# lalitkrajendran/photon

Hardware: AMD Instinct MI355X
Metric: Mrays/sec, 1e7-ray 256^3 BOS render (higher is better)
Workload: dtype f32

## Files before the change

photon_amd/csrc/device_volume_coop.hpp:

```cpp
#pragma once
#include "../../include/photon_philox.h"
#include "device_volume.hpp"

namespace photon {

enum PathSlot : int {
    PS_C_COHERENT,
    PS_C_HIT_CELL,
    PS_C_CELL_IN_TILE,
    PS_C_FETCH_UP,
    PS_C_FETCH_DOWN,
    PS_C_TILE_CLAMPED,
    PS_C_INCOHERENT,
    PS_C_INCOHERENT_LANES,
    PS_C_BRICK_PASS,
    PS_C_BRICK_FETCH,
    PS_C_BRICK_REUSED,
    PS_C_BRICK_CLAMPED,
    PS_C_BRICK_LANES,
    PS_C_GATHER_LANES,
    PS_C_SPIN_OUTSIDE,
    PS_C_SPIN_LOW,
    PS_C_SPIN_CAP,
    PS_L_COHERENT,
    PS_L_HIT_A,
    PS_L_HIT_B,
    PS_L_TILE_B_LANES,
    PS_L_FETCH,
    PS_L_FETCH_TWO,
    PS_L_FETCH_TO_B,
    PS_L_FETCH_DOWN,
    PS_L_BASE_AHEAD,
    PS_L_BASE_BEHIND,
    PS_L_TILE_CLAMPED,
    PS_L_NO_FREE_TILE,
    PS_L_OUT_OF_REACH,
    PS_L_MARK_INCOHERENT,
    PS_L_TILES_SKIPPED,
    PS_L_RETRY,
    PS_L_COHERENT_AGAIN,
    PS_L_INCOHERENT,
    PS_L_INCOHERENT_LANES,
    PS_L_BRICK_PASS,
    PS_L_BRICK_FETCH,
    PS_L_BRICK_REUSED,
    PS_L_BRICK_CLAMPED,
    PS_L_BRICK_LANES,
    PS_L_GATHER_LANES,
    PS_L_SPIN_OUTSIDE,
    PS_L_SPIN_CAP,
    PS_L_LOW,
    PS_L_REPAIR_LANES,
    PS_L_KEEP_PREV_LANES,
    PS_COUNT
};
constexpr int kPathSlots = PS_COUNT;
#ifndef PHOTON_PATH_STATS
#define PHOTON_PATH_STATS 0
#endif
#if PHOTON_PATH_STATS
__device__ unsigned long long g_path_stats[kPathSlots];
__device__ __forceinline__ void path_stat(PathSlot k, unsigned long long n = 1) {
    if ((int)(threadIdx.x & 63) == __ffsll((long long)ballot(true)) - 1) atomicAdd(&g_path_stats[k], n);
}
__device__ __forceinline__ void path_stat_if(PathSlot k, bool c) { if (c) path_stat(k); }
__device__ __forceinline__ void path_lanes(PathSlot k, unsigned long long mask) { if (mask != 0) path_stat(k, (unsigned long long)__popcll(mask)); }
#else
#define path_stat(...) ((void)0)
#define path_stat_if(...) ((void)0)
#define path_lanes(...) ((void)0)
#endif

#ifndef PHOTON_BRICK_PASSES
#define PHOTON_BRICK_PASSES 6
#endif
#ifndef PHOTON_LINEAR_TILE_LAYERS
#define PHOTON_LINEAR_TILE_LAYERS 16
#endif
#ifndef PHOTON_LINEAR_TILES
#define PHOTON_LINEAR_TILES 2
#endif
#ifndef PHOTON_TILE_RETRY_MASK
#define PHOTON_TILE_RETRY_MASK 15
#endif
#ifndef PHOTON_BRICK_PITCH
#define PHOTON_BRICK_PITCH 12
#endif
constexpr int kBrickPitch = PHOTON_BRICK_PITCH;
constexpr int kBrickSlab = 8 * kBrickPitch;
#ifndef PHOTON_CUBIC_TILE_LAYERS
#define PHOTON_CUBIC_TILE_LAYERS 7
#endif
constexpr int kCubicTileLayers = PHOTON_CUBIC_TILE_LAYERS;
static_assert(kCubicTileLayers >= 4 && kCubicTileLayers <= 8, "PHOTON_CUBIC_TILE_LAYERS");
template <int INTERP> constexpr int tile_texels() { return INTERP == 2 ? 16 * kCubicTileLayers : PHOTON_LINEAR_TILES * PHOTON_LINEAR_TILE_LAYERS * 4; }
#ifndef PHOTON_SPINS_IN_LDS
#define PHOTON_SPINS_IN_LDS 1
#endif
constexpr int kSpinSlotTexels = PHOTON_SPINS_IN_LDS ? 32 : 0;
template <int INTERP> constexpr int wave_lds_texels() { return tile_texels<INTERP>() + (INTERP == 2 ? 4 : 2) * kBrickSlab + (INTERP == 1 ? kSpinSlotTexels : 0); }
constexpr int kWaveLdsTexels = wave_lds_texels<2>();

template <int RS, int SS>
__device__ __forceinline__ f4 cubic_taps_lds(const f4 *blk, const float (&wx)[4], const float (&wy)[4],
                                             const float (&wz)[4]) {
    float wxy[4][4];
#pragma unroll
    for (int b = 0; b < 4; b++)
#pragma unroll
        for (int a = 0; a < 4; a++) wxy[b][a] = wx[a] * wy[b];
    f4 acc = f4{0, 0, 0, 0}, s = f4{0, 0, 0, 0};
    float w0 = wxy[0][0];
    f4 t[4];
#pragma unroll
    for (int a = 0; a < 4; a++) t[a] = ldtexel(blk + a);
#pragma unroll
    for (int r = 0; r < 16; r++) {
        const int b = r & 3, c = r >> 2;
#pragma unroll
        for (int a = 0; a < 4; a++) {
            const f4 ta = t[a];
            const float w = (a == 0 && b == 0) ? w0 : wxy[b][a];
            if (a == 0 && b == 0) s = f4{w * ta.x, w * ta.y, w * ta.z, w * ta.w};
            else s = f4{fmaf(w, ta.x, s.x), fmaf(w, ta.y, s.y), fmaf(w, ta.z, s.z), fmaf(w, ta.w, s.w)};
            asm volatile("" : "+v"(s.x), "+v"(s.y), "+v"(s.z), "+v"(s.w) : : "memory");
            if (r < 15) t[a] = ldtexel(blk + ((r + 1) >> 2) * SS + ((r + 1) & 3) * RS + a);
            asm volatile("" : "+v"(w0) : : "memory");
        }
        if (b == 3) {
            if (c == 0) acc = f4{wz[0] * s.x, wz[0] * s.y, wz[0] * s.z, wz[0] * s.w};
            else acc = f4{fmaf(wz[c], s.x, acc.x), fmaf(wz[c], s.y, acc.y), fmaf(wz[c], s.z, acc.z), fmaf(wz[c], s.w, acc.w)};
            asm volatile("" : "+v"(acc.x), "+v"(acc.y), "+v"(acc.z), "+v"(acc.w) : : "memory");
        }
    }
    return acc;
}

#define PH_DPP_ROW0 \
    "v_mul_f32_dpp %0, %8, %12 row_newbcast:0 row_mask:0xf bank_mask:0xf\n\t" \
    "v_mul_f32_dpp %1, %9, %12 row_newbcast:0 row_mask:0xf bank_mask:0xf\n\t" \
    "v_mul_f32_dpp %2, %10, %12 row_newbcast:0 row_mask:0xf bank_mask:0xf\n\t" \
    "v_mul_f32_dpp %3, %11, %12 row_newbcast:0 row_mask:0xf bank_mask:0xf\n\t" \
    "v_fmac_f32_dpp %0, %8, %13 row_newbcast:1 row_mask:0xf bank_mask:0xf\n\t" \
    "v_fmac_f32_dpp %1, %9, %13 row_newbcast:1 row_mask:0xf bank_mask:0xf\n\t" \
    "v_fmac_f32_dpp %2, %10, %13 row_newbcast:1 row_mask:0xf bank_mask:0xf\n\t" \
    "v_fmac_f32_dpp %3, %11, %13 row_newbcast:1 row_mask:0xf bank_mask:0xf\n\t" \
    "v_fmac_f32_dpp %0, %8, %14 row_newbcast:2 row_mask:0xf bank_mask:0xf\n\t" \
    "v_fmac_f32_dpp %1, %9, %14 row_newbcast:2 row_mask:0xf bank_mask:0xf\n\t" \
    "v_fmac_f32_dpp %2, %10, %14 row_newbcast:2 row_mask:0xf bank_mask:0xf\n\t" \
    "v_fmac_f32_dpp %3, %11, %14 row_newbcast:2 row_mask:0xf bank_mask:0xf\n\t" \
    "v_fmac_f32_dpp %0, %8, %15 row_newbcast:3 row_mask:0xf bank_mask:0xf\n\t" \
    "v_fmac_f32_dpp %1, %9, %15 row_newbcast:3 row_mask:0xf bank_mask:0xf\n\t" \
    "v_fmac_f32_dpp %2, %10, %15 row_newbcast:3 row_mask:0xf bank_mask:0xf\n\t" \
    "v_fmac_f32_dpp %3, %11, %15 row_newbcast:3 row_mask:0xf bank_mask:0xf\n\t"
#define PH_DPP_ROW1 \
    "v_fmac_f32_dpp %0, %8, %16 row_newbcast:4 row_mask:0xf bank_mask:0xf\n\t" \
    "v_fmac_f32_dpp %1, %9, %16 row_newbcast:4 row_mask:0xf bank_mask:0xf\n\t" \
    "v_fmac_f32_dpp %2, %10, %16 row_newbcast:4 row_mask:0xf bank_mask:0xf\n\t" \
    "v_fmac_f32_dpp %3, %11, %16 row_newbcast:4 row_mask:0xf bank_mask:0xf\n\t" \
    "v_fmac_f32_dpp %0, %8, %17 row_newbcast:5 row_mask:0xf bank_mask:0xf\n\t" \
    "v_fmac_f32_dpp %1, %9, %17 row_newbcast:5 row_mask:0xf bank_mask:0xf\n\t" \
    "v_fmac_f32_dpp %2, %10, %17 row_newbcast:5 row_mask:0xf bank_mask:0xf\n\t" \
    "v_fmac_f32_dpp %3, %11, %17 row_newbcast:5 row_mask:0xf bank_mask:0xf\n\t" \
    "v_fmac_f32_dpp %0, %8, %18 row_newbcast:6 row_mask:0xf bank_mask:0xf\n\t" \
    "v_fmac_f32_dpp %1, %9, %18 row_newbcast:6 row_mask:0xf bank_mask:0xf\n\t" \
    "v_fmac_f32_dpp %2, %10, %18 row_newbcast:6 row_mask:0xf bank_mask:0xf\n\t" \
    "v_fmac_f32_dpp %3, %11, %18 row_newbcast:6 row_mask:0xf bank_mask:0xf\n\t" \
    "v_fmac_f32_dpp %0, %8, %19 row_newbcast:7 row_mask:0xf bank_mask:0xf\n\t" \
    "v_fmac_f32_dpp %1, %9, %19 row_newbcast:7 row_mask:0xf bank_mask:0xf\n\t" \
    "v_fmac_f32_dpp %2, %10, %19 row_newbcast:7 row_mask:0xf bank_mask:0xf\n\t" \
    "v_fmac_f32_dpp %3, %11, %19 row_newbcast:7 row_mask:0xf bank_mask:0xf\n\t"
#define PH_DPP_ROW2 \
    "v_fmac_f32_dpp %0, %8, %20 row_newbcast:8 row_mask:0xf bank_mask:0xf\n\t" \
    "v_fmac_f32_dpp %1, %9, %20 row_newbcast:8 row_mask:0xf bank_mask:0xf\n\t" \
    "v_fmac_f32_dpp %2, %10, %20 row_newbcast:8 row_mask:0xf bank_mask:0xf\n\t" \
    "v_fmac_f32_dpp %3, %11, %20 row_newbcast:8 row_mask:0xf bank_mask:0xf\n\t" \
    "v_fmac_f32_dpp %0, %8, %21 row_newbcast:9 row_mask:0xf bank_mask:0xf\n\t" \
    "v_fmac_f32_dpp %1, %9, %21 row_newbcast:9 row_mask:0xf bank_mask:0xf\n\t" \
    "v_fmac_f32_dpp %2, %10, %21 row_newbcast:9 row_mask:0xf bank_mask:0xf\n\t" \
    "v_fmac_f32_dpp %3, %11, %21 row_newbcast:9 row_mask:0xf bank_mask:0xf\n\t" \
    "v_fmac_f32_dpp %0, %8, %22 row_newbcast:10 row_mask:0xf bank_mask:0xf\n\t" \
    "v_fmac_f32_dpp %1, %9, %22 row_newbcast:10 row_mask:0xf bank_mask:0xf\n\t" \
    "v_fmac_f32_dpp %2, %10, %22 row_newbcast:10 row_mask:0xf bank_mask:0xf\n\t" \
    "v_fmac_f32_dpp %3, %11, %22 row_newbcast:10 row_mask:0xf bank_mask:0xf\n\t" \
    "v_fmac_f32_dpp %0, %8, %23 row_newbcast:11 row_mask:0xf bank_mask:0xf\n\t" \
    "v_fmac_f32_dpp %1, %9, %23 row_newbcast:11 row_mask:0xf bank_mask:0xf\n\t" \
    "v_fmac_f32_dpp %2, %10, %23 row_newbcast:11 row_mask:0xf bank_mask:0xf\n\t" \
    "v_fmac_f32_dpp %3, %11, %23 row_newbcast:11 row_mask:0xf bank_mask:0xf\n\t"
#define PH_DPP_ROW3 \
    "v_fmac_f32_dpp %0, %8, %24 row_newbcast:12 row_mask:0xf bank_mask:0xf\n\t" \
    "v_fmac_f32_dpp %1, %9, %24 row_newbcast:12 row_mask:0xf bank_mask:0xf\n\t" \
    "v_fmac_f32_dpp %2, %10, %24 row_newbcast:12 row_mask:0xf bank_mask:0xf\n\t" \
    "v_fmac_f32_dpp %3, %11, %24 row_newbcast:12 row_mask:0xf bank_mask:0xf\n\t" \
    "v_fmac_f32_dpp %0, %8, %25 row_newbcast:13 row_mask:0xf bank_mask:0xf\n\t" \
    "v_fmac_f32_dpp %1, %9, %25 row_newbcast:13 row_mask:0xf bank_mask:0xf\n\t" \
    "v_fmac_f32_dpp %2, %10, %25 row_newbcast:13 row_mask:0xf bank_mask:0xf\n\t" \
    "v_fmac_f32_dpp %3, %11, %25 row_newbcast:13 row_mask:0xf bank_mask:0xf\n\t" \
    "v_fmac_f32_dpp %0, %8, %26 row_newbcast:14 row_mask:0xf bank_mask:0xf\n\t" \
    "v_fmac_f32_dpp %1, %9, %26 row_newbcast:14 row_mask:0xf bank_mask:0xf\n\t" \
    "v_fmac_f32_dpp %2, %10, %26 row_newbcast:14 row_mask:0xf bank_mask:0xf\n\t" \
    "v_fmac_f32_dpp %3, %11, %26 row_newbcast:14 row_mask:0xf bank_mask:0xf\n\t" \
    "v_fmac_f32_dpp %0, %8, %27 row_newbcast:15 row_mask:0xf bank_mask:0xf\n\t" \
    "v_fmac_f32_dpp %1, %9, %27 row_newbcast:15 row_mask:0xf bank_mask:0xf\n\t" \
    "v_fmac_f32_dpp %2, %10, %27 row_newbcast:15 row_mask:0xf bank_mask:0xf\n\t" \
    "v_fmac_f32_dpp %3, %11, %27 row_newbcast:15 row_mask:0xf bank_mask:0xf\n\t"
#define PH_DPP_ROWS_TEXT PH_DPP_ROW0 PH_DPP_ROW1 PH_DPP_ROW2 PH_DPP_ROW3
#define PH_DS_OFF1 "16"
#define PH_DS_OFF2 "32"
#define PH_DS_OFF3 "48"
#ifndef PHOTON_PRIO_BASE
#define PHOTON_PRIO_BASE 1
#endif
#ifndef PHOTON_PRIO_BLEND
#define PHOTON_PRIO_BLEND 0
#endif
#ifndef PHOTON_PRIO_TAPS_DPP
#define PHOTON_PRIO_TAPS_DPP 3
#endif
#ifndef PHOTON_PRIO_TAPS_LDS
#define PHOTON_PRIO_TAPS_LDS 0
#endif
#ifndef PHOTON_PRIO_BRICK
#define PHOTON_PRIO_BRICK 2
#endif
#ifndef PHOTON_DPP_SLABS
#define PHOTON_DPP_SLABS 3
#endif
constexpr int kDppSlabs = PHOTON_DPP_SLABS;
static_assert(kDppSlabs >= 1 && kDppSlabs <= 4, "PHOTON_DPP_SLABS");
#define PH_DPP_OPERANDS(S, T) \
            : "=&v"(S.x), "=&v"(S.y), "=&v"(S.z), "=&v"(S.w), "=&v"(d0), "=&v"(d1), "=&v"(d2), "=&v"(d3) \
            : "v"(T.x), "v"(T.y), "v"(T.z), "v"(T.w), "v"(wxy[0][0]), "v"(wxy[0][1]), "v"(wxy[0][2]), "v"(wxy[0][3]), \
              "v"(wxy[1][0]), "v"(wxy[1][1]), "v"(wxy[1][2]), "v"(wxy[1][3]), "v"(wxy[2][0]), "v"(wxy[2][1]), "v"(wxy[2][2]), \
              "v"(wxy[2][3]), "v"(wxy[3][0]), "v"(wxy[3][1]), "v"(wxy[3][2]), "v"(wxy[3][3]) \
            : "memory"
__device__ __forceinline__ void dpp_slab(f4 &s, const f4 &tex, const float (&wxy)[4][4]) {
    float d0, d1, d2, d3;
    asm volatile("s_nop 4\n\t" PH_DPP_ROWS_TEXT PH_DPP_OPERANDS(s, tex));
}
__device__ __forceinline__ f4 cubic_taps_hybrid(const f4 *blk, const f4 &reg, const f4 (&more)[3], const float (&wx)[4], const float (&wy)[4],
                                                const float (&wz)[4]) {
    typedef float v4f __attribute__((ext_vector_type(4)));
    constexpr int R = 4 * kDppSlabs;
    float wxy[4][4];
#pragma unroll
    for (int b = 0; b < 4; b++)
#pragma unroll
        for (int a = 0; a < 4; a++) wxy[b][a] = wx[a] * wy[b];
    v4f t0, t1, t2, t3;
    f4 s;
    const unsigned lds = (unsigned)(size_t)blk + 64u * R;
#if PHOTON_PRIO_TAPS_DPP != PHOTON_PRIO_BASE
    __builtin_amdgcn_s_setprio(PHOTON_PRIO_TAPS_DPP);
#endif
    if (R < 16)
    asm volatile(
            "ds_read_b128 %4, %28\n\t"
            "ds_read_b128 %5, %28 offset:" PH_DS_OFF1 "\n\t"
            "ds_read_b128 %6, %28 offset:" PH_DS_OFF2 "\n\t"
            "ds_read_b128 %7, %28 offset:" PH_DS_OFF3 "\n\t"
            "s_nop 4\n\t"
            PH_DPP_ROWS_TEXT
            "s_waitcnt lgkmcnt(0)"
            : "=&v"(s.x), "=&v"(s.y), "=&v"(s.z), "=&v"(s.w), "=&v"(t0), "=&v"(t1), "=&v"(t2), "=&v"(t3)
            : "v"(reg.x), "v"(reg.y), "v"(reg.z), "v"(reg.w), "v"(wxy[0][0]), "v"(wxy[0][1]), "v"(wxy[0][2]), "v"(wxy[0][3]),
              "v"(wxy[1][0]), "v"(wxy[1][1]), "v"(wxy[1][2]), "v"(wxy[1][3]), "v"(wxy[2][0]), "v"(wxy[2][1]), "v"(wxy[2][2]),
              "v"(wxy[2][3]), "v"(wxy[3][0]), "v"(wxy[3][1]), "v"(wxy[3][2]), "v"(wxy[3][3]), "v"(lds)
            : "memory");
    else {
        dpp_slab(s, reg, wxy);
        t0 = t1 = t2 = t3 = v4f{0, 0, 0, 0};
    }
    f4 acc = f4{wz[0] * s.x, wz[0] * s.y, wz[0] * s.z, wz[0] * s.w};
#pragma unroll
    for (int z = 1; z < kDppSlabs; z++) {
        dpp_slab(s, more[z - 1], wxy);
        acc = f4{fmaf(wz[z], s.x, acc.x), fmaf(wz[z], s.y, acc.y), fmaf(wz[z], s.z, acc.z), fmaf(wz[z], s.w, acc.w)};
        asm volatile("" : "+v"(acc.x), "+v"(acc.y), "+v"(acc.z), "+v"(acc.w) : : "memory");
    }
#if PHOTON_PRIO_TAPS_DPP != PHOTON_PRIO_TAPS_LDS
    __builtin_amdgcn_s_setprio(PHOTON_PRIO_TAPS_LDS);
#endif
    f4 t[4] = {f4{t0.x, t0.y, t0.z, t0.w}, f4{t1.x, t1.y, t1.z, t1.w}, f4{t2.x, t2.y, t2.z, t2.w}, f4{t3.x, t3.y, t3.z, t3.w}};
    float w0 = wxy[0][0];
#pragma unroll
    for (int r = R; r < 16; r++) {
        const int b = r & 3, c = r >> 2;
#pragma unroll
        for (int a = 0; a < 4; a++) {
            const f4 ta = t[a];
            const float w = (a == 0 && b == 0) ? w0 : wxy[b][a];
            if (a == 0 && b == 0) s = f4{w * ta.x, w * ta.y, w * ta.z, w * ta.w};
            else s = f4{fmaf(w, ta.x, s.x), fmaf(w, ta.y, s.y), fmaf(w, ta.z, s.z), fmaf(w, ta.w, s.w)};
            asm volatile("" : "+v"(s.x), "+v"(s.y), "+v"(s.z), "+v"(s.w) : : "memory");
            if (r < 15) t[a] = ldtexel(blk + ((r + 1) >> 2) * 16 + ((r + 1) & 3) * 4 + a);
            asm volatile("" : "+v"(w0) : : "memory");
        }
        if (b == 3) {
            if (c == 0) acc = f4{wz[0] * s.x, wz[0] * s.y, wz[0] * s.z, wz[0] * s.w};
            else acc = f4{fmaf(wz[c], s.x, acc.x), fmaf(wz[c], s.y, acc.y), fmaf(wz[c], s.z, acc.z), fmaf(wz[c], s.w, acc.w)};
            asm volatile("" : "+v"(acc.x), "+v"(acc.y), "+v"(acc.z), "+v"(acc.w) : : "memory");
        }
    }
#if PHOTON_PRIO_TAPS_LDS != PHOTON_PRIO_BASE
    __builtin_amdgcn_s_setprio(PHOTON_PRIO_BASE);
#endif
    return acc;
}

__device__ __forceinline__ bool lane_of(unsigned long long mask) { return __builtin_amdgcn_inverse_ballot_w64(mask); }

struct Parked { int ti, tj, tk; int bi, bj, bk; f4 reg; int ci, cj, k0, coff; int ui, uj, uk; f4 more[3]; };
__device__ __forceinline__ Parked parked_none() {
    return Parked{0x7fffffff, 0x7fffffff, 0x7fffffff, 0x7fffffff, 0x7fffffff, 0x7fffffff, f4{0, 0, 0, 0}, 0x7fffffff, 0x7fffffff, 0, 0, 0x7fffffff, 0x7fffffff, 0x7fffffff, {f4{0, 0, 0, 0}, f4{0, 0, 0, 0}, f4{0, 0, 0, 0}}};
}

struct Lead { int i, j, k; };
__device__ __forceinline__ Lead lead_of(unsigned long long todo, float fi, float fj, float fk) {
    const int leader = __ffsll((long long)todo) - 1;
    return Lead{__builtin_amdgcn_readlane(__float_as_int(fi), leader), __builtin_amdgcn_readlane(__float_as_int(fj), leader),
                __builtin_amdgcn_readlane(__float_as_int(fk), leader)};
}
__device__ __forceinline__ unsigned long long same_block(const Lead &c, float fi, float fj, float fk) {
    return ballot(__float_as_int(fi) == c.i) & ballot(__float_as_int(fj) == c.j) & ballot(__float_as_int(fk) == c.k);
}

__device__ __forceinline__ f4 tex3d_cubic_coop(const VolumeDev &v, const f4 *__restrict__ tex, f4 *blk, unsigned long long need,
                                               float x, float y, float z, Parked &parked) {
    f4 *const brick = blk + tile_texels<2>();
    const float xg = x - 0.5f, yg = y - 0.5f, zg = z - 0.5f;
    const float fi = floorf(xg), fj = floorf(yg), fk = floorf(zg);
    float wx[4], wy[4], wz[4];
    bspline_weights(xg - fi, wx[0], wx[1], wx[2], wx[3]);
    bspline_weights(yg - fj, wy[0], wy[1], wy[2], wy[3]);
    bspline_weights(zg - fk, wz[0], wz[1], wz[2], wz[3]);
    const int lane = threadIdx.x & 63;
    if (need == 0) return f4{0, 0, 0, 0};
    {
        constexpr int TL = kCubicTileLayers;
        bool hit = false;
        if (parked.ti != 0x7fffffff) {
            asm volatile("");
            hit = ((ballot(__float_as_int(fi) == parked.ti) & ballot(__float_as_int(fj) == parked.tj) & ballot(__float_as_int(fk) == parked.tk)) & need) == need;
            path_stat_if(PS_C_HIT_CELL, hit);
        }
        if (!hit) {
            const Lead c = lead_of(need, fi, fj, fk);
            if ((same_block(c, fi, fj, fk) & need) == need) {
                const int ck = (int)__int_as_float(c.k);
                int dz = ck - parked.k0;
                if (c.i != parked.ci || c.j != parked.cj || (unsigned)dz > (unsigned)(TL - 4)) {
                    const int ci = (int)__int_as_float(c.i), cj = (int)__int_as_float(c.j);
                    const bool down = c.i == parked.ci && c.j == parked.cj && dz < 0;
                    const int k0 = down ? ck - (TL - 4) : ck;
                    path_stat(down ? PS_C_FETCH_DOWN : PS_C_FETCH_UP);
                    path_stat_if(PS_C_TILE_CLAMPED, ci < 1 || ci + 2 > v.nx - 1 || cj < 1 || cj + 2 > v.ny - 1 || k0 < 1 || k0 + TL - 2 > v.nz - 1);
                    __builtin_amdgcn_wave_barrier();
                    int l = lane;
                    asm volatile("" : "+v"(l));
                    const int tx = clampi(ci - 1 + (l & 3), 0, v.nx - 1), ty = clampi(cj - 1 + ((l >> 2) & 3), 0, v.ny - 1);
#pragma unroll
                    for (int j = 0; j < (TL + 3) / 4; j++) {
                        if (TL % 4 == 0 || j < TL / 4 || l < 16 * (TL % 4)) {
                            const int tz = clampi(k0 - 1 + (l >> 4) + 4 * j, 0, v.nz - 1);
                            const f4 t = ldtexel(tex + (unsigned)((tz * v.ny + ty) * v.nx + tx));
                            *reinterpret_cast<float4 *>(blk + l + 64 * j) = make_float4(t.x, t.y, t.z, t.w);
                        }
                    }
                    __builtin_amdgcn_wave_barrier();
                    parked.ci = c.i; parked.cj = c.j; parked.k0 = k0;
                    dz = ck - k0;
                } else {
                    path_stat(PS_C_CELL_IN_TILE);
                }
                parked.coff = dz * 16;
                parked.reg = ldtexel(blk + parked.coff + (lane & 15));
#pragma unroll
                for (int z = 1; z < kDppSlabs; z++) parked.more[z - 1] = ldtexel(blk + parked.coff + 16 * z + (lane & 15));
                parked.ti = c.i; parked.tj = c.j; parked.tk = c.k;
                hit = true;
            }
        }
        if (hit) {
            path_stat(PS_C_COHERENT);
            const f4 *cell = blk + parked.coff;
            const f4 acc = cubic_taps_hybrid(cell, parked.reg, parked.more, wx, wy, wz);
            __builtin_amdgcn_wave_barrier();
            return acc;
        }
        parked.ti = 0x7fffffff;
    }
    const int bi = (int)fi, bj = (int)fj, bk = (int)fk;
    f4 acc = f4{0, 0, 0, 0};
    bool done = !lane_of(need);
    unsigned long long todo = need;
    path_stat(PS_C_INCOHERENT);
    path_lanes(PS_C_INCOHERENT_LANES, need);
#pragma unroll 1
    for (int pass = 0; pass < PHOTON_BRICK_PASSES && todo != 0; pass++) {
        const int leader = __ffsll((long long)todo) - 1;
        const int ci = __builtin_amdgcn_readlane(bi, leader), cj = __builtin_amdgcn_readlane(bj, leader),
                  ck = __builtin_amdgcn_readlane(bk, leader);
        const int di = bi - ci + 2, dj = bj - cj + 2;
        const bool in_brick = !done && bk == ck && (unsigned)di <= 4u && (unsigned)dj <= 4u;
        path_stat(PS_C_BRICK_PASS);
        path_lanes(PS_C_BRICK_LANES, ballot(in_brick));
        path_stat(ci != parked.bi || cj != parked.bj || ck != parked.bk ? PS_C_BRICK_FETCH : PS_C_BRICK_REUSED);
        if (ci != parked.bi || cj != parked.bj || ck != parked.bk) {
            path_stat_if(PS_C_BRICK_CLAMPED, ci < 3 || ci + 4 > v.nx - 1 || cj < 3 || cj + 4 > v.ny - 1 || ck < 1 || ck + 2 > v.nz - 1);
            __builtin_amdgcn_wave_barrier();
            int l = lane;
            asm volatile("" : "+v"(l));
            const int slot = (l & 7) + ((l >> 3) & 7) * kBrickPitch;
#pragma unroll
            for (int j = 0; j < 4; j++) {
                const int t = l + 64 * j;
                const int tx = clampi(ci - 3 + (t & 7), 0, v.nx - 1), ty = clampi(cj - 3 + ((t >> 3) & 7), 0, v.ny - 1),
                          tz = clampi(ck - 1 + (t >> 6), 0, v.nz - 1);
                const f4 tv = ldtexel(tex + (unsigned)((tz * v.ny + ty) * v.nx + tx));
                *reinterpret_cast<float4 *>(brick + slot + j * kBrickSlab) = make_float4(tv.x, tv.y, tv.z, tv.w);
            }
            __builtin_amdgcn_wave_barrier();
            parked.bi = ci; parked.bj = cj; parked.bk = ck;
        }
        if (in_brick) {
#if PHOTON_PRIO_BRICK != PHOTON_PRIO_BASE
            __builtin_amdgcn_s_setprio(PHOTON_PRIO_BRICK);
#endif
            acc = cubic_taps_lds<kBrickPitch, kBrickSlab>(brick + (dj * kBrickPitch + di), wx, wy, wz);
#if PHOTON_PRIO_BRICK != PHOTON_PRIO_BASE
            __builtin_amdgcn_s_setprio(PHOTON_PRIO_BASE);
#endif
            done = true;
        }
        __builtin_amdgcn_wave_barrier();
        todo = ballot(!done);
    }
    path_lanes(PS_C_GATHER_LANES, ballot(!done));
    if (!done) acc = cubic_gather_fn(tex, v.nx, v.ny, v.nz, x, y, z);
    return acc;
}

__device__ __attribute__((noinline)) f4 linear_gather_fn(const f4 *__restrict__ tex, int nx, int ny, int nz, float x,
                                                         float y, float z, float weight_scale, float weight_inv) {
    const float xb = x - 0.5f, yb = y - 0.5f, zb = z - 0.5f;
    const float fi = floorf(xb), fj = floorf(yb), fk = floorf(zb);
    const float a = quant_weight(xb - fi, weight_scale, weight_inv), b = quant_weight(yb - fj, weight_scale, weight_inv),
                c = quant_weight(zb - fk, weight_scale, weight_inv);
    const int i = (int)fi, j = (int)fj, k = (int)fk;
    const int i0 = clampi(i, 0, nx - 1), i1 = clampi(i + 1, 0, nx - 1);
    const int j0 = clampi(j, 0, ny - 1), j1 = clampi(j + 1, 0, ny - 1);
    const int k0 = clampi(k, 0, nz - 1), k1 = clampi(k + 1, 0, nz - 1);
    auto row = [&](int kk, int jj) {
        const f4 *r = tex + (unsigned)((kk * ny + jj) * nx);
        f4 v = lerp4(ldtexel(r + i0), ldtexel(r + i1), a);
        asm volatile("" : "+v"(v.x), "+v"(v.y), "+v"(v.z), "+v"(v.w));
        return v;
    };
    const f4 c00 = row(k0, j0), c10 = row(k0, j1);
    f4 c0 = lerp4(c00, c10, b);
    asm volatile("" : "+v"(c0.x), "+v"(c0.y), "+v"(c0.z), "+v"(c0.w));
    const f4 c01 = row(k1, j0), c11 = row(k1, j1);
    const f4 c1 = lerp4(c01, c11, b);
    return lerp4(c0, c1, c);
}

__device__ __forceinline__ float uniformf(float x) {
    float s;
    asm("s_nop 0\n\tv_readfirstlane_b32 %0, %1\n\ts_nop 4" : "=s"(s) : "v"(x));
    return s;
}

__device__ __forceinline__ float pair_swap(float v) {
    return __int_as_float(__builtin_amdgcn_update_dpp(0, __float_as_int(v), 0xB1 , 0xF, 0xF, false));
}

template <bool QUANT, bool PIN = false>
__device__ __forceinline__ f4 tex3d_linear_coop(const VolumeDev &v, const f4 *__restrict__ tex, f4 *blk, unsigned long long need,
                                                float x, float y, float z, Parked &parked, unsigned tick = 0) {
    f4 *const brick = blk + tile_texels<1>();
    const float xb = x - 0.5f, yb = y - 0.5f, zb = z - 0.5f;
    const float fi = floorf(xb), fj = floorf(yb), fk = floorf(zb);
    float a = xb - fi, b = yb - fj, c = zb - fk;
    if (QUANT) {
        a = floorf(fmaf(a, v.weight_scale, 0.5f)) * v.weight_inv;

        b = floorf(fmaf(b, v.weight_scale, 0.5f)) * v.weight_inv;
        c = floorf(fmaf(c, v.weight_scale, 0.5f)) * v.weight_inv;
    }
    const int lane = threadIdx.x & 63;
    if (need == 0) return f4{0, 0, 0, 0};
    {
        constexpr int TL = PHOTON_LINEAR_TILE_LAYERS;
        constexpr int NT = PHOTON_LINEAR_TILES;
        static_assert(TL == 4 || TL == 8 || TL == 16, "PHOTON_LINEAR_TILE_LAYERS");
        static_assert(NT == 1 || NT == 2, "PHOTON_LINEAR_TILES");
        constexpr unsigned kDzMax = (unsigned)(TL - 2);
        constexpr int kIncoherent = 0x7ffffffe;
        const int fib = __float_as_int(fi), fjb = __float_as_int(fj);
        unsigned dzq = 0;
        unsigned long long ok_a = 0, ok_b = 0;
        bool hit = false;
        if (parked.ti != 0x7fffffff) {
            asm volatile("");
            dzq = (unsigned)(int)(fk - __int_as_float(parked.tk));
            ok_a = ballot(fib == parked.ti) & ballot(fjb == parked.tj) & ballot(dzq <= kDzMax);
            hit = (ok_a & need) == need;
            path_stat_if(PS_L_HIT_A, hit);
            if (NT == 2 && !hit && parked.ui < kIncoherent) {
                const unsigned dzu = (unsigned)(int)(fk - __int_as_float(parked.uk));
                ok_b = ballot(fib == parked.ui) & ballot(fjb == parked.uj) & ballot(dzu <= kDzMax);
                if (((ok_a | ok_b) & need) == need) {
                    hit = true;
                    path_stat(PS_L_HIT_B);
                    dzq = lane_of(ok_a) ? dzq : dzu + TL;
                }
            }
        }
        path_stat_if(PS_L_TILES_SKIPPED, !hit && parked.ui == kIncoherent && (tick & (unsigned)PHOTON_TILE_RETRY_MASK) != 0);
        path_stat_if(PS_L_RETRY, !hit && parked.ui == kIncoherent && (tick & (unsigned)PHOTON_TILE_RETRY_MASK) == 0);
        if (!hit && (parked.ui != kIncoherent || (tick & (unsigned)PHOTON_TILE_RETRY_MASK) == 0)) {
            const unsigned long long rest = need & ~(ok_a | ok_b);
            const Lead l1 = lead_of(rest, fi, fj, fk);
            const unsigned long long col1 = rest & ballot(fib == l1.i) & ballot(fjb == l1.j), rest2 = rest & ~col1;
            Lead l2 = l1;
            unsigned long long col2 = 0;
            int n_new = 1;
            if (rest2 != 0) {
                l2 = lead_of(rest2, fi, fj, fk);
                col2 = rest2 & ballot(fib == l2.i) & ballot(fjb == l2.j);
                n_new = (rest2 & ~col2) != 0 ? 3 : 2;
            }
            const bool free_a = (ok_a & need) == 0, free_b = NT == 2 && (ok_b & need) == 0;
            path_stat_if(PS_L_NO_FREE_TILE, n_new > (free_a ? 1 : 0) + (free_b ? 1 : 0));
            if (n_new <= (free_a ? 1 : 0) + (free_b ? 1 : 0)) {
                path_stat_if(PS_L_FETCH_TWO, n_new == 2);
#pragma unroll 1
                for (int j = 0; j < n_new; j++) {
                    path_stat(PS_L_FETCH);
                    const bool to_a = j == 0 && free_a;
                    const Lead ld = j == 0 ? l1 : l2;
                    const unsigned long long lanes = j == 0 ? col1 : col2;
                    const int oi = to_a ? parked.ti : parked.ui, oj = to_a ? parked.tj : parked.uj, ok = to_a ? parked.tk : parked.uk;
                    const float klf = __int_as_float(ld.k);
                    const bool behind = (lanes & ballot(fk < klf)) != 0, ahead = (lanes & ballot(fk > klf)) != 0;
                    const bool down = ld.i == oi && ld.j == oj && klf < __int_as_float(ok);
                    const int ci = (int)__int_as_float(ld.i), cj = (int)__int_as_float(ld.j);
                    const int base = (int)klf - (down ? (ahead ? TL - 3 : TL - 2) : (behind ? 1 : 0));
                    f4 *const tile = blk + (to_a ? 0 : 4 * TL);
                    path_stat_if(PS_L_FETCH_TO_B, !to_a);
                    path_stat_if(PS_L_FETCH_DOWN, down);
                    path_stat_if(PS_L_BASE_AHEAD, down && ahead);
                    path_stat_if(PS_L_BASE_BEHIND, !down && behind);
                    path_stat_if(PS_L_TILE_CLAMPED, ci < 0 || ci + 1 > v.nx - 1 || cj < 0 || cj + 1 > v.ny - 1 || base < 0 || base + TL - 1 > v.nz - 1);
                    __builtin_amdgcn_wave_barrier();
                    if (lane < 4 * TL) {
                        int l = lane;
                        if (PIN) asm volatile("" : "+v"(l));
                        const int tx = clampi(ci + (l & 1), 0, v.nx - 1), ty = clampi(cj + ((l >> 1) & 1), 0, v.ny - 1),
                                  tz = clampi(base + (l >> 2), 0, v.nz - 1);
                        const f4 t = ldtexel(tex + (unsigned)((tz * v.ny + ty) * v.nx + tx));
                        const f4 o = f4{pair_swap(t.x), pair_swap(t.y), pair_swap(t.z), pair_swap(t.w)};
                        const bool hi = (l & 1) != 0;
                        *reinterpret_cast<float4 *>(tile + l) = make_float4(hi ? t.x - o.x : t.x, hi ? t.y - o.y : t.y,
                                                                            hi ? t.z - o.z : t.z, hi ? t.w - o.w : t.w);
                    }
                    __builtin_amdgcn_wave_barrier();
                    const int basef = __float_as_int(uniformf((float)base));
                    if (to_a) { parked.ti = ld.i; parked.tj = ld.j; parked.tk = basef; }
                    else { parked.ui = ld.i; parked.uj = ld.j; parked.uk = basef; }
                }
                dzq = (unsigned)(int)(fk - __int_as_float(parked.tk));
                ok_a = ballot(fib == parked.ti) & ballot(fjb == parked.tj) & ballot(dzq <= kDzMax);
                if (NT == 2 && parked.ui < kIncoherent) {
                    const unsigned dzu = (unsigned)(int)(fk - __int_as_float(parked.uk));
                    ok_b = ballot(fib == parked.ui) & ballot(fjb == parked.uj) & ballot(dzu <= kDzMax);
                    dzq = lane_of(ok_a) ? dzq : dzu + TL;
                }
                hit = ((ok_a | ok_b) & need) == need;
                path_stat_if(PS_L_OUT_OF_REACH, !hit);
                path_stat_if(PS_L_COHERENT_AGAIN, hit && parked.ui == kIncoherent);
                if (hit && parked.ui == kIncoherent) parked.ui = 0x7fffffff;
            }
        }
        if (hit) {
            path_stat(PS_L_COHERENT);
            path_lanes(PS_L_TILE_B_LANES, need & ~ok_a);
            const f4 *q = blk + ((dzq & (unsigned)(NT * TL - 1)) << 2);
#if PHOTON_PRIO_BLEND != PHOTON_PRIO_BASE
            __builtin_amdgcn_s_setprio(PHOTON_PRIO_BLEND);
#endif
            const f4 c00 = lerp4d(ldtexel(q), ldtexel(q + 1), a), c10 = lerp4d(ldtexel(q + 2), ldtexel(q + 3), a);
            const f4 c01 = lerp4d(ldtexel(q + 4), ldtexel(q + 5), a), c11 = lerp4d(ldtexel(q + 6), ldtexel(q + 7), a);
            const f4 c0 = lerp4(c00, c10, b), c1 = lerp4(c01, c11, b);
            const f4 acc = lerp4(c0, c1, c);
#if PHOTON_PRIO_BLEND != PHOTON_PRIO_BASE
            __builtin_amdgcn_s_setprio(PHOTON_PRIO_BASE);
#endif
            __builtin_amdgcn_wave_barrier();
            return acc;
        }
        path_stat_if(PS_L_MARK_INCOHERENT, parked.ui != kIncoherent);
        parked.ti = 0x7fffffff;
        parked.ui = kIncoherent;
    }
    const int bi = (int)fi, bj = (int)fj, bk = (int)fk;
    f4 acc = f4{0, 0, 0, 0};
    bool done = !lane_of(need);
    unsigned long long todo = need;
    path_stat(PS_L_INCOHERENT);
    path_lanes(PS_L_INCOHERENT_LANES, need);
#pragma unroll 1
    for (int pass = 0; pass < PHOTON_BRICK_PASSES && todo != 0; pass++) {
        const int leader = __ffsll((long long)todo) - 1;
        const int ci = __builtin_amdgcn_readlane(bi, leader), cj = __builtin_amdgcn_readlane(bj, leader),
                  ck = __builtin_amdgcn_readlane(bk, leader);
        const int di = bi - ci + 3, dj = bj - cj + 3;
        const bool in_brick = !done && bk == ck && (unsigned)di <= 6u && (unsigned)dj <= 6u;
        path_stat(PS_L_BRICK_PASS);
        path_lanes(PS_L_BRICK_LANES, ballot(in_brick));
        path_stat(ci != parked.bi || cj != parked.bj || ck != parked.bk ? PS_L_BRICK_FETCH : PS_L_BRICK_REUSED);
        if (ci != parked.bi || cj != parked.bj || ck != parked.bk) {
            path_stat_if(PS_L_BRICK_CLAMPED, ci < 3 || ci + 4 > v.nx - 1 || cj < 3 || cj + 4 > v.ny - 1 || ck < 0 || ck + 1 > v.nz - 1);
            __builtin_amdgcn_wave_barrier();
            int l = lane;
            asm volatile("" : "+v"(l));
            const int slot = (l & 7) + ((l >> 3) & 7) * kBrickPitch;
#pragma unroll
            for (int j = 0; j < 2; j++) {
                const int t = l + 64 * j;
                const int tx = clampi(ci - 3 + (t & 7), 0, v.nx - 1), ty = clampi(cj - 3 + ((t >> 3) & 7), 0, v.ny - 1),
                          tz = clampi(ck + (t >> 6), 0, v.nz - 1);
                const f4 tv = ldtexel(tex + (unsigned)((tz * v.ny + ty) * v.nx + tx));
                *reinterpret_cast<float4 *>(brick + slot + j * kBrickSlab) = make_float4(tv.x, tv.y, tv.z, tv.w);
            }
            __builtin_amdgcn_wave_barrier();
            parked.bi = ci; parked.bj = cj; parked.bk = ck;
        }
        if (in_brick) {
#if PHOTON_PRIO_BLEND != PHOTON_PRIO_BASE
            __builtin_amdgcn_s_setprio(PHOTON_PRIO_BLEND);
#endif
            const f4 *q = brick + (dj * kBrickPitch + di);
            const f4 c00 = lerp4(ldtexel(q), ldtexel(q + 1), a), c10 = lerp4(ldtexel(q + kBrickPitch), ldtexel(q + kBrickPitch + 1), a);
            const f4 c01 = lerp4(ldtexel(q + kBrickSlab), ldtexel(q + kBrickSlab + 1), a),
                     c11 = lerp4(ldtexel(q + kBrickSlab + kBrickPitch), ldtexel(q + kBrickSlab + kBrickPitch + 1), a);
            const f4 c0 = lerp4(c00, c10, b), c1 = lerp4(c01, c11, b);
            acc = lerp4(c0, c1, c);
#if PHOTON_PRIO_BLEND != PHOTON_PRIO_BASE
            __builtin_amdgcn_s_setprio(PHOTON_PRIO_BASE);
#endif
            done = true;
        }
        __builtin_amdgcn_wave_barrier();
        todo = ballot(!done);
    }
    path_lanes(PS_L_GATHER_LANES, ballot(!done));
    if (!done) acc = linear_gather_fn(tex, v.nx, v.ny, v.nz, x, y, z, v.weight_scale, v.weight_inv);
    return acc;
}

struct MarchU {
    float minx, miny, minz, maxx, maxy, maxz;
    float sx, sy, sz;
    float nxm2, nym2, nzm2;
    float fnx, fny, fnz;
    float step, data_min, spin_step;
    int nx, ny, nz;
};
__device__ __forceinline__ MarchU make_march_consts(const VolumeDev &v, f3 scale) {
    MarchU u;
    u.minx = uniformf(v.min_bound.x); u.miny = uniformf(v.min_bound.y); u.minz = uniformf(v.min_bound.z);
    u.maxx = uniformf(v.max_bound.x); u.maxy = uniformf(v.max_bound.y); u.maxz = uniformf(v.max_bound.z);
    u.sx = uniformf(scale.x); u.sy = uniformf(scale.y); u.sz = uniformf(scale.z);
    u.nxm2 = uniformf((float)(v.nx - 2)); u.nym2 = uniformf((float)(v.ny - 2)); u.nzm2 = uniformf((float)(v.nz - 2));
    u.fnx = uniformf((float)v.nx); u.fny = uniformf((float)v.ny); u.fnz = uniformf((float)v.nz);
    u.step = uniformf(v.step_size); u.data_min = uniformf(v.data_min);
    u.spin_step = uniformf(v.step_size / (1 + v.data_min));
    u.nx = v.nx; u.ny = v.ny; u.nz = v.nz;
    return u;
}
__device__ __forceinline__ f3 lookup_index_u(f3 pos, const MarchU &u) {
    const f3 off = mk3(pos.x - u.minx, pos.y - u.miny, pos.z - u.minz);
    const f3 fn = mk3(u.sx * off.x, u.sy * off.y, u.sz * off.z);
    return mk3(1 + fn.x * u.nxm2, 1 + fn.y * u.nym2, 1 + fn.z * u.nzm2);
}
__device__ __forceinline__ unsigned long long access_mask(const MarchU &u, f3 l) {
    return ~(ballot(l.x < 0) | ballot(l.y < 0) | ballot(l.z < 0) | ballot(l.x >= u.fnx) | ballot(l.y >= u.fny) | ballot(l.z >= u.fnz));
}
__device__ __forceinline__ unsigned long long inside_mask(f3 p, const MarchU &u) {
    return ~(ballot(p.x < u.minx) | ballot(p.y < u.miny) | ballot(p.z < u.minz) | ballot(p.x >= u.maxx) | ballot(p.y >= u.maxy) | ballot(p.z >= u.maxz));
}

struct WaveCount { unsigned iterations; unsigned samples; };
__device__ __forceinline__ void count_samples(MarchCount &mc, unsigned long long m) { if (lane_of(m)) mc.samples++; }
__device__ __forceinline__ void count_iterations(MarchCount &mc, unsigned long long m) { if (lane_of(m)) mc.iterations++; }
__device__ __forceinline__ void count_samples(WaveCount &mc, unsigned long long m) { mc.samples += (unsigned)__popcll(m); }
__device__ __forceinline__ void count_iterations(WaveCount &mc, unsigned long long m) { mc.iterations += (unsigned)__popcll(m); }

struct PrevVal {
    f4 v;
    __device__ __forceinline__ void init(f4 *, f4 x) { v = x; }
    __device__ __forceinline__ void set(f4 x) { v = x; }
    __device__ __forceinline__ f4 get() const { return v; }
};

template <int INTERP, bool QUANT, class CNT, bool PIN = false>
__device__ __forceinline__ f4 sample_coop(const VolumeDev &v, const f4 *__restrict__ tex, f4 *blk, unsigned long long need, f3 lookup,
                                          const PrevVal &prev, float data_min, CNT &mc, Parked &parked, unsigned tick = 0) {
    f4 val = INTERP == 1 ? tex3d_linear_coop<QUANT, PIN>(v, tex, blk, need, lookup.x, lookup.y, lookup.z, parked, tick)
                         : tex3d_cubic_coop(v, tex, blk, need, lookup.x, lookup.y, lookup.z, parked);
    count_samples(mc, need);
    if (INTERP == 1) {
        const unsigned long long low = need & ballot(val.w < data_min);
        if (low != 0) {
            const float ambient = 1.000277;
            const f4 val_prev = prev.get();
            const unsigned long long repair = low & ballot(val_prev.w == 0);
            path_stat(PS_L_LOW);
            path_lanes(PS_L_REPAIR_LANES, repair);
            path_lanes(PS_L_KEEP_PREV_LANES, low & ~repair);
            if (repair != 0) {
                count_samples(mc, repair);
                if (lane_of(repair)) {
                    const f4 t = linear_gather_fn(tex, v.nx, v.ny, v.nz, lookup.x, lookup.y, lookup.z - 1, v.weight_scale, v.weight_inv);
                    val = f4{t.x, t.y, t.z, ambient - 1};
                }
            }
            if (lane_of(low & ~repair)) val = val_prev;
        }
    }
    return val;
}

struct MarchResume {
    int loop_ctr, spins;
    f4 val_prev;
    unsigned max_trips;
    unsigned trips_base;
    bool fresh;
// ... 195 lines not shown
```

photon_amd/path_stats.py:

```python
from __future__ import annotations

import ctypes
import os
import re

HEADER = os.path.join(os.path.dirname(os.path.abspath(__file__)), "csrc", "device_volume_coop.hpp")

SLOTS = (
    "C_COHERENT", "C_HIT_CELL", "C_CELL_IN_TILE", "C_FETCH_UP", "C_FETCH_DOWN", "C_TILE_CLAMPED",
    "C_INCOHERENT", "C_INCOHERENT_LANES", "C_BRICK_PASS", "C_BRICK_FETCH", "C_BRICK_REUSED", "C_BRICK_CLAMPED",
    "C_BRICK_LANES", "C_GATHER_LANES", "C_SPIN_OUTSIDE", "C_SPIN_LOW", "C_SPIN_CAP",
    "L_COHERENT", "L_HIT_A", "L_HIT_B", "L_TILE_B_LANES", "L_FETCH", "L_FETCH_TWO", "L_FETCH_TO_B", "L_FETCH_DOWN",
    "L_BASE_AHEAD", "L_BASE_BEHIND", "L_TILE_CLAMPED", "L_NO_FREE_TILE", "L_OUT_OF_REACH", "L_MARK_INCOHERENT",
    "L_TILES_SKIPPED", "L_RETRY", "L_COHERENT_AGAIN", "L_INCOHERENT", "L_INCOHERENT_LANES", "L_BRICK_PASS",
    "L_BRICK_FETCH", "L_BRICK_REUSED", "L_BRICK_CLAMPED", "L_BRICK_LANES", "L_GATHER_LANES", "L_SPIN_OUTSIDE",
    "L_SPIN_CAP", "L_LOW", "L_REPAIR_LANES", "L_KEEP_PREV_LANES",
)

OPTICS_HEADER = os.path.join(os.path.dirname(os.path.abspath(__file__)), "csrc", "device_optics.hpp")

SPLAT_SLOTS = (
    "E_WAVES", "E_COOP", "E_FALLBACK", "E_FB_WIDE", "E_FB_TILES", "E_FB_RADIUS",
    "E_SHARED_X_LANES", "E_BOTH_X_LANES", "E_SHARED_Y_LANES", "E_BOTH_Y_LANES", "E_CLIPPED_LANES", "E_LANE_CLIPPED_LANES",
    "E_TILES", "E_TILES_SAME", "E_TILES_MIXED", "E_MULTI_TILE",
    "T_WAVES", "T_COOP", "T_LANE_ROUTE", "T_MULTI_TILE", "T_TAPS_LANDED", "T_TAPS_DROPPED", "T_TAPS_WRAPPED",
    "K_GEN_ERF", "K_STATE_ERF", "K_GEN_TRAIN", "K_STATE_TRAIN", "K_GEN_TAPS", "K_STATE_TAPS",
)

PATH_STATS_FLAGS = ("-DPHOTON_PATH_STATS=1",)


def header_slots(path: str = HEADER):
    with open(path) as f:
        text = f.read()
    body = re.search(r"enum PathSlot\s*:\s*int\s*\{(.*?)\};", text, re.S).group(1)
    names = re.findall(r"^\s*PS_(\w+)\s*,", body, re.M)
    assert names and names[-1] != "COUNT"
    return tuple(names)


def header_splat_slots(path: str = OPTICS_HEADER):
    with open(path) as f:
        text = f.read()
    body = re.search(r"enum SplatSlot\s*:\s*int\s*\{(.*?)\};", text, re.S).group(1)
    names = re.findall(r"^\s*SS_(\w+)\s*,", body, re.M)
    assert names and names[-1] != "COUNT"
    return tuple(names)


def read_splat(lib) -> dict:
    f = lib.lib.photon_debug_splat_stats
    f.argtypes = [ctypes.c_void_p, ctypes.c_int]
    f.restype = ctypes.c_int
    out = (ctypes.c_ulonglong * len(SPLAT_SLOTS))()
    rc = f(ctypes.cast(out, ctypes.c_void_p), len(SPLAT_SLOTS))
    if rc != 0:
        raise RuntimeError(f"photon_debug_splat_stats failed ({rc})")
    return dict(zip(SPLAT_SLOTS, (int(v) for v in out)))


def read(lib) -> dict:
    f = lib.lib.photon_debug_path_stats
    f.argtypes = [ctypes.c_void_p, ctypes.c_int]
    f.restype = ctypes.c_int
    out = (ctypes.c_ulonglong * len(SLOTS))()
    rc = f(ctypes.cast(out, ctypes.c_void_p), len(SLOTS))
    if rc != 0:
        raise RuntimeError(f"photon_debug_path_stats failed ({rc})")
    return dict(zip(SLOTS, (int(v) for v in out)))
```

Before: 189.3.

## Serve split cubic waves from two cached LDS tiles instead of brick passes

Factors the cubic tile fetch into a reusable helper and adds a second cached 4x4xTL tile (stored in the brick region, tagged in parked.bi/bj/bk). When an incoherent wave's lanes fall into exactly two cells that are contiguous by lane and at most one z-layer apart, each lane evaluates its taps from tile A or tile B in LDS, skipping the brick-pass loop. The aim is to avoid repeated brick fetches and the global gather fallback for waves that straddle a cell boundary. In exchange it adds extra ballots and leader reads on every incoherent call, and it reuses the brick LDS slab, which may evict cached brick state.

```diff
diff --git a/photon_amd/csrc/device_volume_coop.hpp b/photon_amd/csrc/device_volume_coop.hpp
--- a/photon_amd/csrc/device_volume_coop.hpp
+++ b/photon_amd/csrc/device_volume_coop.hpp
@@ -11,6 +11,9 @@
     PS_C_FETCH_UP,
     PS_C_FETCH_DOWN,
     PS_C_TILE_CLAMPED,
+    PS_C_TWO_TILES,
+    PS_C_TILE_B_FETCH,
+    PS_C_TILE_B_LANES,
     PS_C_INCOHERENT,
     PS_C_INCOHERENT_LANES,
     PS_C_BRICK_PASS,
@@ -93,6 +96,7 @@
 #endif
 constexpr int kCubicTileLayers = PHOTON_CUBIC_TILE_LAYERS;
 static_assert(kCubicTileLayers >= 4 && kCubicTileLayers <= 8, "PHOTON_CUBIC_TILE_LAYERS");
+constexpr int kTileBTag = 0x40000000;
 template <int INTERP> constexpr int tile_texels() { return INTERP == 2 ? 16 * kCubicTileLayers : PHOTON_LINEAR_TILES * PHOTON_LINEAR_TILE_LAYERS * 4; }
 #ifndef PHOTON_SPINS_IN_LDS
 #define PHOTON_SPINS_IN_LDS 1
@@ -325,6 +329,36 @@
     return ballot(__float_as_int(fi) == c.i) & ballot(__float_as_int(fj) == c.j) & ballot(__float_as_int(fk) == c.k);
 }
 
+__device__ __forceinline__ int cubic_tile_seek(const VolumeDev &v, const f4 *__restrict__ tex, f4 *tile, int lane, const Lead &c,
+                                               int &pci, int &pcj, int &pk0, int &how) {
+    constexpr int TL = kCubicTileLayers;
+    const int ck = (int)__int_as_float(c.k);
+    int dz = ck - pk0;
+    how = 0;
+    if (c.i != pci || c.j != pcj || (unsigned)dz > (unsigned)(TL - 4)) {
+        const int ci = (int)__int_as_float(c.i), cj = (int)__int_as_float(c.j);
+        const bool down = c.i == pci && c.j == pcj && dz < 0;
+        const int k0 = down ? ck - (TL - 4) : ck;
+        how = (down ? 2 : 1) | (ci < 1 || ci + 2 > v.nx - 1 || cj < 1 || cj + 2 > v.ny - 1 || k0 < 1 || k0 + TL - 2 > v.nz - 1 ? 4 : 0);
+        __builtin_amdgcn_wave_barrier();
+        int l = lane;
+        asm volatile("" : "+v"(l));
+        const int tx = clampi(ci - 1 + (l & 3), 0, v.nx - 1), ty = clampi(cj - 1 + ((l >> 2) & 3), 0, v.ny - 1);
+#pragma unroll
+        for (int j = 0; j < (TL + 3) / 4; j++) {
+            if (TL % 4 == 0 || j < TL / 4 || l < 16 * (TL % 4)) {
+                const int tz = clampi(k0 - 1 + (l >> 4) + 4 * j, 0, v.nz - 1);
+                const f4 t = ldtexel(tex + (unsigned)((tz * v.ny + ty) * v.nx + tx));
+                *reinterpret_cast<float4 *>(tile + l + 64 * j) = make_float4(t.x, t.y, t.z, t.w);
+            }
+        }
+        __builtin_amdgcn_wave_barrier();
+        pci = c.i; pcj = c.j; pk0 = k0;
+        dz = ck - k0;
+    }
+    return dz * 16;
+}
+
 __device__ __forceinline__ f4 tex3d_cubic_coop(const VolumeDev &v, const f4 *__restrict__ tex, f4 *blk, unsigned long long need,
                                                float x, float y, float z, Parked &parked) {
     f4 *const brick = blk + tile_texels<2>();
@@ -337,7 +371,6 @@
     const int lane = threadIdx.x & 63;
     if (need == 0) return f4{0, 0, 0, 0};
     {
-        constexpr int TL = kCubicTileLayers;
         bool hit = false;
         if (parked.ti != 0x7fffffff) {
             asm volatile("");
@@ -347,33 +380,10 @@
         if (!hit) {
             const Lead c = lead_of(need, fi, fj, fk);
             if ((same_block(c, fi, fj, fk) & need) == need) {
-                const int ck = (int)__int_as_float(c.k);
-                int dz = ck - parked.k0;
-                if (c.i != parked.ci || c.j != parked.cj || (unsigned)dz > (unsigned)(TL - 4)) {
-                    const int ci = (int)__int_as_float(c.i), cj = (int)__int_as_float(c.j);
-                    const bool down = c.i == parked.ci && c.j == parked.cj && dz < 0;
-                    const int k0 = down ? ck - (TL - 4) : ck;
-                    path_stat(down ? PS_C_FETCH_DOWN : PS_C_FETCH_UP);
-                    path_stat_if(PS_C_TILE_CLAMPED, ci < 1 || ci + 2 > v.nx - 1 || cj < 1 || cj + 2 > v.ny - 1 || k0 < 1 || k0 + TL - 2 > v.nz - 1);
-                    __builtin_amdgcn_wave_barrier();
-                    int l = lane;
-                    asm volatile("" : "+v"(l));
-                    const int tx = clampi(ci - 1 + (l & 3), 0, v.nx - 1), ty = clampi(cj - 1 + ((l >> 2) & 3), 0, v.ny - 1);
-#pragma unroll
-                    for (int j = 0; j < (TL + 3) / 4; j++) {
-                        if (TL % 4 == 0 || j < TL / 4 || l < 16 * (TL % 4)) {
-                            const int tz = clampi(k0 - 1 + (l >> 4) + 4 * j, 0, v.nz - 1);
-                            const f4 t = ldtexel(tex + (unsigned)((tz * v.ny + ty) * v.nx + tx));
-                            *reinterpret_cast<float4 *>(blk + l + 64 * j) = make_float4(t.x, t.y, t.z, t.w);
-                        }
-                    }
-                    __builtin_amdgcn_wave_barrier();
-                    parked.ci = c.i; parked.cj = c.j; parked.k0 = k0;
-                    dz = ck - k0;
-                } else {
-                    path_stat(PS_C_CELL_IN_TILE);
-                }
-                parked.coff = dz * 16;
+                int how;
+                parked.coff = cubic_tile_seek(v, tex, blk, lane, c, parked.ci, parked.cj, parked.k0, how);
+                path_stat(how == 0 ? PS_C_CELL_IN_TILE : (how & 2) ? PS_C_FETCH_DOWN : PS_C_FETCH_UP);
+                path_stat_if(PS_C_TILE_CLAMPED, (how & 4) != 0);
                 parked.reg = ldtexel(blk + parked.coff + (lane & 15));
 #pragma unroll
                 for (int z = 1; z < kDppSlabs; z++) parked.more[z - 1] = ldtexel(blk + parked.coff + 16 * z + (lane & 15));
@@ -394,10 +404,44 @@
     f4 acc = f4{0, 0, 0, 0};
     bool done = !lane_of(need);
     unsigned long long todo = need;
-    path_stat(PS_C_INCOHERENT);
-    path_lanes(PS_C_INCOHERENT_LANES, need);
+    const Lead ca = lead_of(need, fi, fj, fk);
+    const unsigned long long in_a = same_block(ca, fi, fj, fk) & need;
+    const Lead cb = lead_of(need & ~in_a, fi, fj, fk);
+    const unsigned long long in_b = same_block(cb, fi, fj, fk) & need;
+    const bool two = PHOTON_BRICK_PASSES > 0 && (in_a | in_b) == need && (in_a & ((need & ~in_a) | (0 - (need & ~in_a)))) == 0 &&
+                     (unsigned)((int)__int_as_float(cb.k) - (int)__int_as_float(ca.k) + 1) <= 2u;
+    const f4 *cell = blk;
+    if (two) {
+        int how_a, how_b;
+        int mine_b = lane_of(in_b) ? 1 : 0;
+        asm volatile("" : "+v"(mine_b));
+        const int off_a = cubic_tile_seek(v, tex, blk, lane, ca, parked.ci, parked.cj, parked.k0, how_a);
+        int bk0 = parked.bk - kTileBTag;
+        const int off_b = cubic_tile_seek(v, tex, brick, lane, cb, parked.bi, parked.bj, bk0, how_b);
+        parked.bk = bk0 + kTileBTag;
+        path_stat(PS_C_TWO_TILES);
+        path_stat_if(PS_C_TILE_B_FETCH, how_b != 0);
+        path_stat_if(PS_C_TILE_CLAMPED, ((how_a | how_b) & 4) != 0);
+        path_lanes(PS_C_TILE_B_LANES, in_b);
+        cell = mine_b != 0 ? brick + off_b : blk + off_a;
+    }
+    if (!two) {
+        path_stat(PS_C_INCOHERENT);
+        path_lanes(PS_C_INCOHERENT_LANES, need);
+    }
 #pragma unroll 1
     for (int pass = 0; pass < PHOTON_BRICK_PASSES && todo != 0; pass++) {
+        if (two) {
+#if PHOTON_PRIO_BRICK != PHOTON_PRIO_BASE
+            __builtin_amdgcn_s_setprio(PHOTON_PRIO_BRICK);
+#endif
+            acc = cubic_taps_lds<4, 16>(cell, wx, wy, wz);
+#if PHOTON_PRIO_BRICK != PHOTON_PRIO_BASE
+            __builtin_amdgcn_s_setprio(PHOTON_PRIO_BASE);
+#endif
+            __builtin_amdgcn_wave_barrier();
+            break;
+        }
         const int leader = __ffsll((long long)todo) - 1;
         const int ci = __builtin_amdgcn_readlane(bi, leader), cj = __builtin_amdgcn_readlane(bj, leader),
                   ck = __builtin_amdgcn_readlane(bk, leader);
@@ -436,6 +480,7 @@
         __builtin_amdgcn_wave_barrier();
         todo = ballot(!done);
     }
+    if (two) done = true;
     path_lanes(PS_C_GATHER_LANES, ballot(!done));
     if (!done) acc = cubic_gather_fn(tex, v.nx, v.ny, v.nz, x, y, z);
     return acc;
diff --git a/photon_amd/path_stats.py b/photon_amd/path_stats.py
--- a/photon_amd/path_stats.py
+++ b/photon_amd/path_stats.py
@@ -8,6 +8,7 @@
 
 SLOTS = (
     "C_COHERENT", "C_HIT_CELL", "C_CELL_IN_TILE", "C_FETCH_UP", "C_FETCH_DOWN", "C_TILE_CLAMPED",
+    "C_TWO_TILES", "C_TILE_B_FETCH", "C_TILE_B_LANES",
     "C_INCOHERENT", "C_INCOHERENT_LANES", "C_BRICK_PASS", "C_BRICK_FETCH", "C_BRICK_REUSED", "C_BRICK_CLAMPED",
     "C_BRICK_LANES", "C_GATHER_LANES", "C_SPIN_OUTSIDE", "C_SPIN_LOW", "C_SPIN_CAP",
     "L_COHERENT", "L_HIT_A", "L_HIT_B", "L_TILE_B_LANES", "L_FETCH", "L_FETCH_TWO", "L_FETCH_TO_B", "L_FETCH_DOWN",
```

Result: no change. 190.2 (median of 6 runs) (+0.5%).
